# UNC-CFD/somar

Hardware: AMD Instinct MI355X
Metric: pressure-Poisson V-cycles/sec (higher is better)
Workload: dtype f64; 1 GPU; C2 single-level 512^3 Poisson, diagonal stretched metric, Neumann, LevelGSRB V-cycle 2/2/2 + BiCGStab bottom; layout = 1 box(es) 512x512x512, one per GPU; mg_depth=8, cells=134217728

## Files before the change

somar_amd/build.py:

```python
import os
import subprocess
import sys

HERE = os.path.dirname(os.path.abspath(__file__))
CSRC = os.path.join(HERE, "csrc")
OUT = os.path.join(HERE, "libsomar_amd.so")
SOURCES = ["kernels.hip", "box_bicgstab.hip", "gsrb_fused.hip", "resid_march.hip", "full19.hip", "full19_march.hip", "full19_fused.hip", "projection.hip", "line_gsrb.hip", "amr_kernels.hip", "leptic_kernels.hip", "maps.hip", "metric_refresh.hip", "box_io.hip", "tuning.cpp", "level.cpp", "solver.cpp", "solver_full.cpp", "amr.cpp", "leptic.cpp", "comm_rccl.cpp", "comm_shm.cpp", "capi.cpp"]
HEADERS = ["common.h", "devbuf.h", "tuning.h", "kernels.h", "level.h", "solver.h", "amr.h", "leptic.h", os.path.join("..", "..", "include", "somar_amd.h")]
HIPCC = os.environ.get("HIPCC", "/opt/rocm/bin/hipcc")
FLAGS = ["--offload-arch=gfx950", "-O3", "-std=c++17", "-fPIC", "-ffp-contract=off", "-fno-fast-math",
         "-Wall", "-Wno-unused-result", "-Wno-unused-value", "-I/opt/rocm/include"]


EXTRA = os.environ.get("SOMAR_EXTRA_FLAGS", "").split()


def _stale():
    if not os.path.exists(OUT):
        return True
    t = os.path.getmtime(OUT)
    return any(os.path.getmtime(os.path.join(CSRC, f)) > t for f in SOURCES + HEADERS)


def build(force=False, verbose=False):
    if not (force or _stale()):
        return OUT
    objs = []
    for f in SOURCES:
        src = os.path.join(CSRC, f)
        obj = os.path.join(CSRC, os.path.splitext(f)[0] + ".o")
        cmd = [HIPCC] + FLAGS + EXTRA + (["-x", "hip"] if f.endswith(".cpp") else []) + ["-c", src, "-o", obj]
        if verbose:
            print(" ".join(cmd))
        subprocess.check_call(cmd)
        objs.append(obj)
    cmd = [HIPCC, "--offload-arch=gfx950", "-shared", "-fPIC", "-o", OUT] + objs + ["-ldl", "-lrt"]
    if verbose:
        print(" ".join(cmd))
    subprocess.check_call(cmd)
    return OUT


if __name__ == "__main__":
    print(build(force="--force" in sys.argv, verbose=True))
```

somar_amd/csrc/gsrb_fused.hip:

```cpp
#include <type_traits>

#include "common.h"
#include "kernels.h"

namespace somar {


template <class T>
__device__ __forceinline__ T pick(const typename Vec2<T>::type& v, int s) { return s ? v.y : v.x; }

template <class T>
__device__ __forceinline__ typename Vec2<T>::type ld2(const T* __restrict__ a, long long idx, bool ok0, bool ok1,
                                                      long long safe)
{
#ifdef SOMAR_NT_LOADS
    typedef T v2d_ __attribute__((ext_vector_type(2)));
    const v2d_ w = __builtin_nontemporal_load(reinterpret_cast<const v2d_*>(a + ((ok0 || ok1) ? idx : safe)));
    const typename Vec2<T>::type v = mk2<T>(w.x, w.y);
#else
    const typename Vec2<T>::type v = *reinterpret_cast<const typename Vec2<T>::type*>(a + ((ok0 || ok1) ? idx : safe));
#endif
    return mk2<T>(ok0 ? v.x : T(0), ok1 ? v.y : T(0));
}

// ... 217 lines not shown
                        if ((p.cf & 32) && kb == p.n[2] - 1) pzh = T(P.cf_c1[2]) * own + T(P.cf_c2[2]) * zl;
                    }
                    black = gsrb_point<DIRI, INT, T>(P, xxS, yyS, zzS, p.lo[0] + li + c, gj, p.lo[2] + kb, pxl, pxh, pyl, pyh,
                                       pzl, pzh, b_gxl, b_gxh, b_gyl, b_gyh, b_gzl, pick<T>(Gzc, c), b_ji, b_rhs,
                                       Sx(sb, row, rc));
                }
                T* dst = phi_out + base + sk * kb;
                const T ox = c ? redPrev1 : black, oy = c ? black : redPrev1;
                if (out_ij[0] && out_ij[1]) *reinterpret_cast<T2*>(dst) = mk2<T>(ox, oy);
                else if (out_ij[0]) dst[0] = ox;
                else dst[1] = oy;
            }
        }

        {
            const int cb = c ^ 1;
            b_rhs = pick<T>(Rh, cb);
            b_ji = pick<T>(Ji, cb);
            b_gxl = cb ? Gx.y : Gx.x;
            b_gxh = cb ? gx_next : Gx.y;
            b_gyl = pick<T>(Gy, cb);
            b_gyh = pick<T>(Gyh, cb);
            b_gzl = pick<T>(Gzc, cb);
        }
        redPrev2 = redPrev1;
        redPrev1 = red;
        Pm = Pc;
        Pc = Pp;
        Gzc = Gzp;
    };
    const int cfirst = __builtin_amdgcn_readfirstlane((p.lo[0] + li + gj + p.lo[2] + k) & 1);
    if (cfirst) {
        for (;;) {
            if (k > kend) break;
            step(std::integral_constant<int, 1>{});
            ++k;
            if (k > kend) break;
            step(std::integral_constant<int, 0>{});
            ++k;
        }
    } else {
        for (;;) {
            if (k > kend) break;
            step(std::integral_constant<int, 0>{});
            ++k;
            if (k > kend) break;
            step(std::integral_constant<int, 1>{});
            ++k;
        }
    }
#undef Sx
}

template <int FR_J, int INMODE, bool DIRI = false, bool UNI = false, bool NARROW = false, class T = double>
__global__ __launch_bounds__(64 * FR_J) void k_gsrb_fused(const Tile* __restrict__ tiles,
                                                     const PatchDesc* __restrict__ patches,
                                                     T* __restrict__ phi_out,
                                                     const T* __restrict__ phi_in,
                                                     const T* __restrict__ rhs,
                                                     const T* __restrict__ jgx,
                                                     const T* __restrict__ jgy,
                                                     const T* __restrict__ jgz,
                                                     const T* __restrict__ jinv, StencilParams P,
                                                     const double* __restrict__ sums,
                                                     const PatchDesc* __restrict__ cpatches,
                                                     const T* __restrict__ crse, int r0, int r1, int r2, int lean_ok)
{
    __shared__ __attribute__((aligned(16))) T S[3 * FR_J * (NARROW ? 160 : 128)];
    const Tile t = tiles[blockIdx.x];
    const PatchDesc p = patches[t.patch];
    const int cls = NARROW ? t.pad_[1] : 0;
    bool lean = false;
    if (UNI && !DIRI) {
        const int wi = t.pad_[0] > 0 ? t.pad_[0] : 124;
        const int ilo = t.i0 - 1, ihi = min(t.i0 + wi, p.n[0]), jlo = t.j0 - 1, jhi = min(t.j0 + (FR_J << cls) - 4, p.n[1]);
        lean = lean_ok && p.lo[0] + ilo > P.dom_lo[0] && p.lo[0] + ihi < P.dom_hi[0] && p.lo[1] + jlo > P.dom_lo[1] &&
               p.lo[1] + jhi < P.dom_hi[1] && !((p.cf & 1) && ilo < 0) && !((p.cf & 2) && ihi >= p.n[0]) &&
               !((p.cf & 4) && jlo < 0) && !((p.cf & 8) && jhi >= p.n[1]);
    }
#define SOMAR_FUSED_BODY(INT_, CLS_)                                                                                          \
    gsrb_fused_body<FR_J, INMODE, DIRI, UNI, INT_, CLS_, T>(S, t, p, phi_out, phi_in, rhs, jgx, jgy, jgz, jinv, P, sums, cpatches, \
                                                        crse, r0, r1, r2)
    if (!NARROW || cls == 0) {
        if (lean) SOMAR_FUSED_BODY(UNI && !DIRI, 0);
        else SOMAR_FUSED_BODY(false, 0);
    } else if (cls == 1) {
        if (lean) SOMAR_FUSED_BODY(UNI && !DIRI, NARROW ? 1 : 0);
        else SOMAR_FUSED_BODY(false, NARROW ? 1 : 0);
    } else {
        SOMAR_FUSED_BODY(false, NARROW ? 4 : 0);
    }
#undef SOMAR_FUSED_BODY
}

template <class T>
static void launch_gsrb_fused_t(hipStream_t st, const Tile* tiles, int ntiles, const LevelDev& L, const MetricPtrs<T>& M,
                                T* phi_out, const T* phi_in, const T* rhs, int in_mode, const double* sums,
                                const LevelDev* C, const T* crse, const int* r)
{
    if (ntiles == 0) return;
    const PatchDesc* cpatches = C ? C->patches : nullptr;
    const int r0 = r ? r[0] : 1, r1 = r ? r[1] : 1, r2 = r ? r[2] : 1;
    SOMAR_CHECK(in_mode < 3 || ((r0 == 1 || r0 == 2) && (r1 == 1 || r1 == 2) && (r2 == 1 || r2 == 2)),
                "internal: the prolongation folded into a sweep takes multigrid ratios of 1 or 2 per direction");
    auto go = [&](auto kern, int rows) {
        hipLaunchKernelGGL(kern, dim3(ntiles), dim3(64, rows, 1), 0, st, tiles, L.patches, phi_out, phi_in, rhs, M.jg[0], M.jg[1],
                           M.jg[2], M.jinv, L.P, sums, cpatches, crse, r0, r1, r2, L.lean_tiles);
    };
#define SOMAR_FUSED_MODES(ROWS, D, U, N, M0, M1, M2, M3, M4)                    \
    switch (in_mode) {                                                          \
        case 1: go(k_gsrb_fused<ROWS, M1, D, U, N, T>, ROWS); break;            \
        case 2: go(k_gsrb_fused<ROWS, M2, D, U, N, T>, ROWS); break;            \
        case 3: go(k_gsrb_fused<ROWS, M3, D, U, N, T>, ROWS); break;            \
        case 4: go(k_gsrb_fused<ROWS, M4, D, U, N, T>, ROWS); break;            \
        default: go(k_gsrb_fused<ROWS, M0, D, U, N, T>, ROWS);                  \
    }
    const bool rows16 = L.fused_rows == 16;
    const bool narrow = L.narrow7 != 0 && rows16;
    bool diri = false;
    for (int d = 0; d < 3; ++d) diri = diri || L.P.diri[d][0] || L.P.diri[d][1];
    if (diri) {
        SOMAR_CHECK(in_mode == 0 || in_mode == 1 || in_mode == 3, "internal: mean removal on a level with Dirichlet sides");
        if (!rows16) { SOMAR_FUSED_MODES(8, true, false, false, 0, 1, 0, 3, 3) }
        else if (narrow) { SOMAR_FUSED_MODES(16, true, false, true, 0, 1, 0, 3, 3) }
        else { SOMAR_FUSED_MODES(16, true, false, false, 0, 1, 0, 3, 3) }
        return;
    }
    if (L.P.uniform && rows16) {
        if (narrow) { SOMAR_FUSED_MODES(16, false, true, true, 0, 1, 2, 3, 4) }
        else { SOMAR_FUSED_MODES(16, false, true, false, 0, 1, 2, 3, 4) }
        return;
    }
    if (!rows16) { SOMAR_FUSED_MODES(8, false, false, false, 0, 1, 2, 3, 4) }
    else if (narrow) { SOMAR_FUSED_MODES(16, false, false, true, 0, 1, 2, 3, 4) }
    else { SOMAR_FUSED_MODES(16, false, false, false, 0, 1, 2, 3, 4) }
#undef SOMAR_FUSED_MODES
}

void launch_gsrb_fused(hipStream_t st, const Tile* tiles, int ntiles, const LevelDev& L, const MetricPtrs<double>& M,
                       double* phi_out, const double* phi_in, const double* rhs, int in_mode, const double* sums,
                       const LevelDev* C, const double* crse, const int* r)
{
    launch_gsrb_fused_t<double>(st, tiles, ntiles, L, M, phi_out, phi_in, rhs, in_mode, sums, C, crse, r);
}

void launch_gsrb_fused(hipStream_t st, const Tile* tiles, int ntiles, const LevelDev& L, const MetricPtrs<float>& M,
                       float* phi_out, const float* phi_in, const float* rhs, int in_mode, const double* sums,
                       const LevelDev* C, const float* crse, const int* r)
{
    SOMAR_CHECK(fused_uniform_kernel(L) || (M.jg[0] && M.jg[1] && M.jg[2] && M.jinv),
                "internal: the fused sweep streams the metric of this depth, but its fp32 copies are missing");
    launch_gsrb_fused_t<float>(st, tiles, ntiles, L, M, phi_out, phi_in, rhs, in_mode, sums, C, crse, r);
}

bool fused_uniform_kernel(const LevelDev& L)
{
    bool diri = false;
    for (int d = 0; d < 3; ++d) diri = diri || L.P.diri[d][0] || L.P.diri[d][1];
    return L.P.uniform && L.fused_rows == 16 && !diri;
}

}
```

somar_amd/csrc/kernels.h:

```cpp
#pragma once
#include "common.h"

namespace somar {

struct LevelDev {
    const Tile* tiles = nullptr;
    int ntiles = 0;
    int tile_j = 4;
    const CopyItem* tile_items = nullptr;
    const int* tile_item_start = nullptr;
    int ghost_gy = 16;
    const PatchDesc* patches = nullptr;
    int npatches = 0;
    double* jg[3] = {nullptr, nullptr, nullptr};
    double* jinv = nullptr;
    double* lapdiag = nullptr;
    double* jgf[3][3] = {{nullptr, nullptr, nullptr}, {nullptr, nullptr, nullptr}, {nullptr, nullptr, nullptr}};
    StencilParams P;
    const double* bc_face = nullptr;
    int narrow7 = 0;
    int narrowq = 0;
    int fused_rows = 16;
    int full_rows = 8;
    int lean_tiles = 1;
    int ordered_serial = 0;
};

template <class T>
struct MetricPtrs { const T* jg[3]; const T* jinv; };
inline MetricPtrs<double> metric_ptrs(const LevelDev& L) { return MetricPtrs<double>{{L.jg[0], L.jg[1], L.jg[2]}, L.jinv}; }

struct FullFlux { const double* psi = nullptr; const double* J[3][3] = {{nullptr, nullptr, nullptr}, {nullptr, nullptr, nullptr}, {nullptr, nullptr, nullptr}}; double dxi[3] = {0, 0, 0}; };

void launch_ghost_ops(hipStream_t st, const LevelDev& L, const GhostOp* ops, int nops, double* phi, double* psi,
                      bool bc_homog = true, bool redirect = false);
void launch_ghost_ops(hipStream_t st, const LevelDev& L, const GhostOp* ops, int nops, float* phi);
void launch_ghost_program(hipStream_t st, const LevelDev& L, const GhostOp* box_ops, const int* box_first, double* phi,
                          double* psi, bool bc_homog, bool redirect, bool copy_all);
void launch_full_march(hipStream_t st, const Tile* tiles, int ntiles, const LevelDev& L, double* out, const double* phi,
                       const double* psi, const double* rhs, int mode);
void launch_gsrb_full_march(hipStream_t st, const Tile* tiles, int ntiles, const LevelDev& L, double* out,
                            const double* phi, const double* psi, const double* rhs, int color);
void launch_full_fused(hipStream_t st, const Tile* tiles, int ntiles, const LevelDev& L, double* out, const double* phi,
                       const double* psi, const double* rhs);
void launch_gsrb_full_shell(hipStream_t st, const Tile* tiles, int ntiles, const LevelDev& L, double* phi, const double* phi_in,
                            const double* psi, const double* rhs);
void launch_flux_full(hipStream_t st, const LevelDev& L, double* const out[3], const double* phi, const double* psi);
void launch_op_full(hipStream_t st, const LevelDev& L, double* out, const double* phi, const double* psi,
                    const double* rhs, int mode);
void launch_gsrb_full(hipStream_t st, const LevelDev& L, double* phi, const double* psi, const double* rhs, int color);

void launch_gsrb_ortho(hipStream_t st, const LevelDev& L, double* phi, const double* rhs, int color, int loose = 0,
                       bool pull = false);
void launch_gsrb_fused(hipStream_t st, const Tile* tiles, int ntiles, const LevelDev& L, const MetricPtrs<double>& M,
                       double* phi_out, const double* phi_in, const double* rhs, int in_mode, const double* sums,
                       const LevelDev* C, const double* crse, const int* r);
void launch_gsrb_fused(hipStream_t st, const Tile* tiles, int ntiles, const LevelDev& L, const MetricPtrs<float>& M,
                       float* phi_out, const float* phi_in, const float* rhs, int in_mode, const double* sums,
                       const LevelDev* C, const float* crse, const int* r);
bool fused_uniform_kernel(const LevelDev& L);
void launch_resid_march(hipStream_t st, const Tile* tiles, int ntiles, const LevelDev& L, double* out,
                        const double* phi, const double* rhs, int mode);
void launch_resid_restrict(hipStream_t st, const Tile* tiles, int ntiles, const LevelDev& F, const MetricPtrs<double>& M,
                           const LevelDev& C, double* crse, const double* phi, const double* rhs, const int r[3],
                           double dxProduct, double* volsum);
void launch_resid_restrict(hipStream_t st, const Tile* tiles, int ntiles, const LevelDev& F, const MetricPtrs<float>& M,
                           const LevelDev& C, float* crse, const float* phi, const float* rhs, const int r[3],
                           double dxProduct, double* volsum);
void launch_child_volume(hipStream_t st, const LevelDev& C, const LevelDev& F, double* crse, const int r[3],
                         double dxProduct);
void launch_sum_partials(hipStream_t st, const double* partials, int n, double* out);
void launch_combine_sums(hipStream_t st, double* out, const double* a, const double* b, const double* c);
void launch_line_gsrb_2d(hipStream_t st, const LevelDev& L, int maxN0, double* phi, const double* rhs, double* dmod, int color,
// ... 141 lines not shown
```

somar_amd/csrc/level.cpp:

```cpp
#include "level.h"

#include <algorithm>
#include <array>
#include <cstdlib>
#include <cstring>

namespace somar {

bool coarsenable(const std::vector<IBox>& boxes, const int* r)
{
    for (const IBox& b : boxes)
        if (!(b.coarsen(r).refine(r) == b)) return false;
    return true;
}

ExchangePlan build_exchange_plan(const IBox& domain, const bool periodic[3], const int ghost[3],
                                 const std::vector<IBox>& boxes, const std::vector<int>& owner, int myrank)
{
    ExchangePlan plan;
    std::vector<std::array<int, 3>> shifts;
    for (int a = -1; a <= 1; ++a)
        for (int b = -1; b <= 1; ++b)
            for (int cc = -1; cc <= 1; ++cc) {
                if ((a && !periodic[0]) || (b && !periodic[1]) || (cc && !periodic[2])) continue;
                shifts.push_back({a * domain.size(0), b * domain.size(1), cc * domain.size(2)});
            }
    struct Remote { int peer; CopyItem it; };
    std::vector<Remote> sends, recvs;
    for (size_t di = 0; di < boxes.size(); ++di) {
        const IBox gbox = boxes[di].grow(ghost);
        for (size_t si = 0; si < boxes.size(); ++si) {
            const bool dl = owner[di] == myrank, sl = owner[si] == myrank;
            if (!dl && !sl) continue;
            for (const auto& sh : shifts) {
                if (si == di && sh[0] == 0 && sh[1] == 0 && sh[2] == 0) continue;
                const IBox img = boxes[si].shift(sh.data());
                const IBox r = gbox & img;
                if (r.empty()) continue;
                CopyItem it;
                std::memset(&it, 0, sizeof(it));
                it.src_patch = (int)si;
                it.dst_patch = (int)di;
                for (int d = 0; d < 3; ++d) {
                    it.n[d] = r.size(d);
                    it.dst_lo[d] = r.lo[d] - boxes[di].lo[d];
                    it.src_lo[d] = r.lo[d] - sh[d] - boxes[si].lo[d];
                }
                if (dl && sl) plan.local.push_back(it);
                else if (sl) sends.push_back({owner[di], it});
                else recvs.push_back({owner[si], it});
            }
        }
    }
// ... 348 lines not shown
        if (owner[b] == myrank) plan.local.push_back(item(b));
    for (int q = 0; q < nranks; ++q) {
        if (q == myrank) continue;
        plan.peers.push_back(q);
        plan.soff.push_back(plan.send_total);
        for (size_t b = 0; b < boxes.size(); ++b)
            if (owner[b] == myrank) {
                const CopyItem it = item(b);
                plan.send_items.push_back(it);
                plan.send_itemoff.push_back(plan.send_total);
                plan.send_total += (long long)it.n[0] * it.n[1] * it.n[2];
            }
        plan.scount.push_back(plan.send_total - plan.soff.back());
        plan.roff.push_back(plan.recv_total);
        for (size_t b = 0; b < boxes.size(); ++b)
            if (owner[b] == q) {
                const CopyItem it = item(b);
                plan.recv_items.push_back(it);
                plan.recv_itemoff.push_back(plan.recv_total);
                plan.recv_total += (long long)it.n[0] * it.n[1] * it.n[2];
            }
        plan.rcount.push_back(plan.recv_total - plan.roff.back());
    }
    return plan;
}

void Copier::define_allgather(const Level& src, const Level& dst, int grow, Comm* comm)
{
    src_ = &src;
    dst_ = &dst;
    comm_ = comm;
    SOMAR_CHECK(grow >= 0 && grow <= FRAME, "allgather: ghost wider than the device frame");
    SOMAR_CHECK(dst.boxes.size() == src.boxes.size() && dst.local.size() == dst.boxes.size(),
                "allgather: the destination layout must hold every box locally");
    plan = build_allgather_plan(src.boxes, src.owner, grow, comm ? comm->rank : 0, comm ? comm->size : 1);
    std::vector<int> sp(src.boxes.size(), -1);
    for (int pi = 0; pi < (int)src.local.size(); ++pi) sp[src.local[pi]] = pi;
    for (CopyItem& it : plan.local) it.src_patch = sp[it.src_patch];
    for (CopyItem& it : plan.send_items) it.src_patch = sp[it.src_patch];
    upload_tables();
}

void Copier::run(const double* s, double* d, hipStream_t st) const
{
    const bool remote = !plan.peers.empty();
    if (remote) {
        launch_pack(st, src_->dev, d_send, d_soff, (int)plan.send_items.size(), const_cast<double*>(s), d_sbuf, true);
        comm_->neighbor_exchange(d_sbuf, d_rbuf, plan.peers, plan.soff, plan.scount, plan.roff, plan.rcount, st);
    }
    launch_copy_items2(st, src_->dev.patches, dst_->dev.patches, d_local, (int)plan.local.size(), s, d);
    if (remote) launch_pack(st, dst_->dev, d_recv, d_roff, (int)plan.recv_items.size(), d, d_rbuf, false);
}

void Level::build_march_tiles(bool narrow7)
{
    for (DevBuf<Tile>* q : {&d_ftiles, &d_ftiles_own, &d_ftiles_rem, &d_rtiles, &d_rtiles_own, &d_rtiles_rem, &d_qtiles, &d_gtiles, &d_stiles})
        q->reset();
    nftiles_own = nftiles_rem = nrtiles_own = nrtiles_rem = 0;
    narrow7_ = narrow7;
    struct ColSpec { int i0, w, cls; };
    const int fused_rows = dev.fused_rows, full_rows = dev.full_rows;
    auto march_tiles = [&](int FT_I, int region_rows, int hrows, double halo, int slots, bool classes, double min_gain = 1.0) {
        classes = classes && !tune.no_narrow_tiles;
        const bool balanced = !tune.no_balanced_tiles;
        auto columns = [&](int n0) {
            std::vector<ColSpec> eq, v;
            {
                int w = FT_I;
                if (balanced) {
                    const int ncol = (n0 + FT_I - 1) / FT_I;
                    w = (n0 + ncol - 1) / ncol;
                    w += w & 1;
                    w = std::min(w, FT_I);
                }
                for (int i0 = 0; i0 < n0; i0 += w) eq.push_back({i0, w, 0});
            }
            if (!classes || (n0 & 1)) return eq;
            int i0 = 0, rem = n0;
            double cost = 0.0;
            while (rem >= FT_I) { v.push_back({i0, FT_I, 0}); i0 += FT_I; rem -= FT_I; cost += 1.0; }
            if (rem > 76) { v.push_back({i0, rem, 0}); rem = 0; cost += 1.0; }
            if (rem > 16) { const int w = std::min(rem, 60); v.push_back({i0, w, 1}); i0 += w; rem -= w; cost += 0.5; }
            while (rem > 0) { const int w = std::min(rem, 4); v.push_back({i0, w, 4}); i0 += w; rem -= w; cost += 0.25; }
            return cost <= min_gain * (double)eq.size() ? v : eq;
        };
        auto rows_of = [&](int cls) { return (region_rows << cls) - hrows; };
        long long cols = 0;
        int maxn2 = 1;
        for (const PatchDesc& p : hpatches) {
            for (const ColSpec& c : columns(p.n[0])) cols += (p.n[1] + rows_of(c.cls) - 1) / rows_of(c.cls);
            maxn2 = std::max(maxn2, p.n[2]);
        }
        int best = 1;
        double best_eff = -1.0;
        for (int nch = 1; nch <= 64 && (nch == 1 || maxn2 / nch >= 4); ++nch) {
            const long long blocks = cols * nch;
            const long long rounds = (blocks + slots - 1) / slots;
            const double nk = (double)maxn2 / nch;
            const double eff = (double)blocks / (double)(rounds * slots) * nk / (nk + halo);
            if (eff > best_eff + 1e-9) { best_eff = eff; best = nch; }
        }
        std::vector<Tile> fnat;
        for (int pi = 0; pi < (int)hpatches.size(); ++pi) {
            const PatchDesc& p = hpatches[pi];
            int nk = (p.n[2] + best - 1) / best;
            nk += nk & 1;
            const std::vector<ColSpec> cs = columns(p.n[0]);
            auto add = [&](const ColSpec& c, int j0, int k0) {
                Tile t;
                std::memset(&t, 0, sizeof(t));
                t.patch = pi; t.i0 = c.i0; t.j0 = j0; t.k0 = k0;
                t.nk = std::min(nk, p.n[2] - k0);
                t.pad_[0] = c.w;
                t.pad_[1] = c.cls;
                fnat.push_back(t);
            };
            for (int k0 = 0; k0 < p.n[2]; k0 += nk) {
                const size_t first = fnat.size();
                for (const ColSpec& c : cs)
                    for (int j0 = 0; j0 < p.n[1]; j0 += rows_of(c.cls)) add(c, j0, k0);
                std::stable_sort(fnat.begin() + first, fnat.end(), [](const Tile& a, const Tile& b) {
                    return a.j0 != b.j0 ? a.j0 < b.j0 : a.i0 < b.i0;
                });
            }
        }
        const int NF = (int)fnat.size();
        std::vector<Tile> perm(NF);
        const int NX = 8;
        int start[NX + 1];
        start[0] = 0;
        for (int x = 0; x < NX; ++x) start[x + 1] = start[x] + (NF - x + NX - 1) / NX;
        for (int b = 0; b < NF; ++b) perm[b] = fnat[start[b % NX] + b / NX];
        return perm;
    };
    hftiles = march_tiles(124, fused_rows, 4, 3.0, 256, narrow7 && fused_rows == 16, 0.85);
    d_ftiles = DevBuf<Tile>::from(hftiles);
    nftiles = (int)hftiles.size();
    hrtiles = march_tiles(124, 16, 2, 2.0, 256, narrow7, 0.85);
    for (size_t q = 0; q < hrtiles.size(); ++q) hrtiles[q].pad_[2] = (int)q;
    d_rtiles = DevBuf<Tile>::from(hrtiles);
    nrtiles = (int)hrtiles.size();
    dev.narrow7 = 0;
    for (const Tile& t : hftiles) if (t.pad_[1]) dev.narrow7 = 1;
    hqtiles = march_tiles(124, full_rows, 2, 2.0, full_rows == 6 ? 512 : 256, full_rows == 8, 0.85);
    d_qtiles = DevBuf<Tile>::from(hqtiles);
    nqtiles = (int)hqtiles.size();
    dev.narrowq = 0;
    for (const Tile& t : hqtiles) if (t.pad_[1]) dev.narrowq = 1;
    ngtiles = nstiles = 0;
    if (want_fused19_) {
        const std::vector<Tile> g = march_tiles(124, 8, 4, 3.0, 256, false);
        d_gtiles = DevBuf<Tile>::from(g);
        ngtiles = (int)g.size();
        std::vector<Tile> sh;
        const int KC = 32;
        for (int pi = 0; pi < (int)hpatches.size(); ++pi) {
            const PatchDesc& p = hpatches[pi];
            auto add = [&](int i0, int w, int cls, int j0, int k0, int nk) {
                Tile t;
                std::memset(&t, 0, sizeof(t));
                t.patch = pi; t.i0 = i0; t.j0 = j0; t.k0 = k0; t.nk = nk;
                t.pad_[0] = w; t.pad_[1] = cls;
                sh.push_back(t);
            };
            int wcol = 124;
            {
                const int ncol = (p.n[0] + 123) / 124;
                wcol = (p.n[0] + ncol - 1) / ncol;
                wcol += wcol & 1;
                wcol = std::min(wcol, 124);
            }
            for (int k0 = 0; k0 < p.n[2]; k0 += KC) {
                const int nk = std::min(KC, p.n[2] - k0);
                for (int xi : {0, std::max(0, p.n[0] - 4)})
                    for (int j0 = 0; j0 < p.n[1]; j0 += 126) add(xi, 4, 4, j0, k0, nk);
                for (int yj : {0, std::max(0, p.n[1] - 6)})
                    for (int i0 = 0; i0 < p.n[0]; i0 += wcol) add(i0, wcol, 0, yj, k0, nk);
            }
            for (int zk : {0, std::max(0, p.n[2] - 3)})
                for (int j0 = 0; j0 < p.n[1]; j0 += 6)
                    for (int i0 = 0; i0 < p.n[0]; i0 += wcol) add(i0, wcol, 0, j0, zk, std::min(3, p.n[2] - zk));
        }
        d_stiles = DevBuf<Tile>::from(sh);
        nstiles = (int)sh.size();
    }

    if (!plan.peers.empty()) {
        std::vector<std::vector<const CopyItem*>> byDst(hpatches.size());
        for (const CopyItem& it : plan.recv_items) byDst[it.dst_patch].push_back(&it);
        auto split = [&](const std::vector<Tile>& all, int region_rows, int hrows, int halo, std::vector<Tile>& own, std::vector<Tile>& rem) {
            for (const Tile& t : all) {
                const PatchDesc& p = hpatches[t.patch];
                const int w = t.pad_[0] > 0 ? t.pad_[0] : 124;
                const int rows = (region_rows << t.pad_[1]) - hrows;
                const int lo[3] = {t.i0 - halo, t.j0 - halo, t.k0 - halo};
                const int hi[3] = {std::min(t.i0 + w, p.n[0]) - 1 + halo, std::min(t.j0 + rows, p.n[1]) - 1 + halo, t.k0 + t.nk - 1 + halo};
// ... 82 lines not shown
        for (int k0 = 0; k0 < p.n[2]; k0 += tk)
            for (int j0 = 0; j0 < p.n[1]; j0 += tj)
                for (int i0 = 0; i0 < p.n[0]; i0 += TILE_I) {
                    Tile t;
                    std::memset(&t, 0, sizeof(t));
                    t.patch = pi; t.i0 = i0; t.j0 = j0; t.k0 = k0;
                    t.nk = std::min(tk, p.n[2] - k0);
                    nat.push_back(t);
                }
    }
    const int N = (int)nat.size();
    htiles.assign(N, Tile());
    {
        const int NX = 8;
        int start[NX + 1];
        start[0] = 0;
        for (int x = 0; x < NX; ++x) start[x + 1] = start[x] + (N - x + NX - 1) / NX;
        for (int b = 0; b < N; ++b) htiles[b] = nat[start[b % NX] + b / NX];
    }

    {
        for (int pi = 0; pi < (int)hpatches.size(); ++pi) {
            const PatchDesc& p = hpatches[pi];
            for (int j0 = 0; j0 < p.n[1]; j0 += ctile_j)
                for (int i0 = 0; i0 < p.n[0]; i0 += TILE_I) {
                    Tile t;
                    std::memset(&t, 0, sizeof(t));
                    t.patch = pi; t.i0 = i0; t.j0 = j0; t.k0 = 0; t.nk = p.n[2];
                    hctiles.push_back(t);
                }
        }
        d_ctiles = DevBuf<Tile>::from(hctiles);
        nctiles = (int)hctiles.size();
    }

    int ghost[3];
    for (int d = 0; d < 3; ++d) ghost[d] = active[d] ? FRAME : 0;
    plan = build_exchange_plan(domain, periodic, ghost, boxes, owner, myrank);
    {
        std::vector<int> patch_of(boxes.size(), -1);
        for (int pi = 0; pi < (int)local.size(); ++pi) patch_of[local[pi]] = pi;
        for (CopyItem& it : plan.local) { it.src_patch = patch_of[it.src_patch]; it.dst_patch = patch_of[it.dst_patch]; }
        for (CopyItem& it : plan.send_items) it.src_patch = patch_of[it.src_patch];
        for (CopyItem& it : plan.recv_items) it.dst_patch = patch_of[it.dst_patch];
    }

    d_patches = DevBuf<PatchDesc>::from(hpatches);
    d_tiles = DevBuf<Tile>::from(htiles);
    d_local_items = DevBuf<CopyItem>::from(plan.local);
    d_send_items = DevBuf<CopyItem>::from(plan.send_items);
    d_recv_items = DevBuf<CopyItem>::from(plan.recv_items);
    d_send_off = DevBuf<long long>::from(plan.send_itemoff);
    d_recv_off = DevBuf<long long>::from(plan.recv_itemoff);
    build_march_tiles(false);
    d_sendbuf = plan.send_total ? DevBuf<double>(plan.send_total) : DevBuf<double>();
    d_recvbuf = plan.recv_total ? DevBuf<double>(plan.recv_total) : DevBuf<double>();

    dev.tiles = d_tiles;
    dev.ntiles = N;
    dev.patches = d_patches;
    dev.npatches = (int)hpatches.size();
    {
        const long long pullMax = tune.pull_max_cells;
        long long cells = 0;
        for (const IBox& b : boxes) cells += b.numPts();
        if (plan.peers.empty() && cells <= pullMax && N > 0) {
            std::vector<std::vector<int>> byDst(hpatches.size());
            for (int q = 0; q < (int)plan.local.size(); ++q) byDst[plan.local[q].dst_patch].push_back(q);
            std::vector<CopyItem> titems;
            std::vector<int> tstart(N + 1, 0);
            for (int b = 0; b < N; ++b) {
                const Tile& t = htiles[b];
                const PatchDesc& p = hpatches[t.patch];
                int lo[3] = {t.i0, t.j0, t.k0};
                int hi[3] = {std::min(t.i0 + TILE_I, p.n[0]) - 1, std::min(t.j0 + dev.tile_j, p.n[1]) - 1, t.k0 + t.nk - 1};
                for (int d = 0; d < 3; ++d)
                    if (active[d]) { lo[d] -= 1; hi[d] += 1; }
                tstart[b] = (int)titems.size();
                for (int q : byDst[t.patch]) {
                    const CopyItem& it = plan.local[q];
                    CopyItem c = it;
                    bool empty = false;
                    for (int d = 0; d < 3; ++d) {
                        const int a = std::max(lo[d], it.dst_lo[d]), e = std::min(hi[d], it.dst_lo[d] + it.n[d] - 1);
                        if (e < a) { empty = true; break; }
                        c.dst_lo[d] = a;
                        c.src_lo[d] = it.src_lo[d] + (a - it.dst_lo[d]);
                        c.n[d] = e - a + 1;
                    }
                    if (!empty) titems.push_back(c);
                }
            }
            tstart[N] = (int)titems.size();
            if (titems.empty()) titems.push_back(CopyItem());
            d_tile_items = DevBuf<CopyItem>::from(titems);
            d_tile_item_start = DevBuf<int>::from(tstart);
            dev.tile_items = d_tile_items;
            dev.tile_item_start = d_tile_item_start;
        }
    }
    {
        long long face = 0;
        for (const PatchDesc& q : hpatches) {
            const long long a = (long long)(q.n[0] + 2 * FRAME), b = (long long)(q.n[1] + 2 * FRAME), c = (long long)(q.n[2] + 2 * FRAME);
            face = std::max(face, std::max(a * b, std::max(a * c, b * c)));
        }
        dev.ghost_gy = (int)std::min<long long>(256, std::max<long long>(16, (face + 1023) / 1024));
// ... 294 lines not shown
```

somar_amd/csrc/level.h:

```cpp
#pragma once
#include <array>
#include <memory>
#include <vector>

#include "common.h"
#include "devbuf.h"
#include "kernels.h"
#include "tuning.h"

namespace somar {

struct IBox {
    int lo[3], hi[3];
    IBox() : lo{0, 0, 0}, hi{-1, -1, -1} {}
    IBox(const int* l, const int* h) { for (int d = 0; d < 3; ++d) { lo[d] = l[d]; hi[d] = h[d]; } }
    bool empty() const { return hi[0] < lo[0] || hi[1] < lo[1] || hi[2] < lo[2]; }
    int size(int d) const { return hi[d] - lo[d] + 1; }
    long long numPts() const { return empty() ? 0 : (long long)size(0) * size(1) * size(2); }
    IBox grow(const int* g) const { IBox b = *this; for (int d = 0; d < 3; ++d) { b.lo[d] -= g[d]; b.hi[d] += g[d]; } return b; }
    IBox shift(const int* s) const { IBox b = *this; for (int d = 0; d < 3; ++d) { b.lo[d] += s[d]; b.hi[d] += s[d]; } return b; }
    IBox operator&(const IBox& o) const {
        IBox b;
        for (int d = 0; d < 3; ++d) { b.lo[d] = lo[d] > o.lo[d] ? lo[d] : o.lo[d]; b.hi[d] = hi[d] < o.hi[d] ? hi[d] : o.hi[d]; }
        return b;
// ... 29 lines not shown
                                   const std::vector<long long>& soff, const std::vector<long long>& scount,
                                   const std::vector<long long>& roff, const std::vector<long long>& rcount,
                                   hipStream_t st)
    {
        (void)sendbuf; (void)recvbuf; (void)peers; (void)soff; (void)scount; (void)roff; (void)rcount; (void)st;
    }
};

struct ExchangePlan {
    std::vector<CopyItem> local;
    std::vector<int> peers;
    std::vector<CopyItem> send_items, recv_items;
    std::vector<long long> send_itemoff, recv_itemoff;
    std::vector<long long> soff, scount, roff, rcount;
    long long send_total = 0, recv_total = 0;
};

ExchangePlan build_exchange_plan(const IBox& domain, const bool periodic[3], const int ghost[3],
                                 const std::vector<IBox>& boxes, const std::vector<int>& owner, int myrank);

struct BoxIoShape {
    int ghost[3] = {0, 0, 0};
    int grow[3] = {0, 0, 0};
    int face = -1;
    int ncomp = 1;
    bool operator==(const BoxIoShape& o) const
    {
        for (int d = 0; d < 3; ++d) if (ghost[d] != o.ghost[d] || grow[d] != o.grow[d]) return false;
        return face == o.face && ncomp == o.ncomp;
    }
    static BoxIoShape cells(const int g[3], bool with_ghosts)
    {
        BoxIoShape s;
        for (int d = 0; d < 3; ++d) { s.ghost[d] = g[d]; s.grow[d] = with_ghosts ? g[d] : 0; }
        return s;
    }
    static BoxIoShape faces(int dir) { BoxIoShape s; s.face = dir; return s; }
};
void check_shape(const BoxIoShape& s);
struct BoxIoBoxes { IBox caller, region; };

class Level {
public:
    IBox domain;
    bool periodic[3] = {false, false, false};
    double dx[3] = {1, 1, 1};
    int active[3] = {1, 1, 1};
    int bc_type[3][2];
    std::vector<IBox> boxes;
    std::vector<int> owner;
    std::vector<int> local;
    std::vector<PatchDesc> hpatches;
    std::vector<Tile> htiles;
    void build_march_tiles(bool narrow7);
    bool narrow7_ = false;
    std::vector<Tile> hftiles;
    DevBuf<Tile> d_ftiles;
    int nftiles = 0;
    DevBuf<Tile> d_ftiles_own, d_ftiles_rem;
    int nftiles_own = 0, nftiles_rem = 0;
    DevBuf<Tile> d_rtiles_own, d_rtiles_rem;
    int nrtiles_own = 0, nrtiles_rem = 0;
    std::vector<Tile> hrtiles;
    DevBuf<Tile> d_rtiles;
    int nrtiles = 0;
    std::vector<Tile> hqtiles;
    DevBuf<Tile> d_qtiles;
    int nqtiles = 0;
    bool want_fused19_ = false;
    DevBuf<Tile> d_gtiles, d_stiles;
    int ngtiles = 0, nstiles = 0;
    std::vector<Tile> hctiles;
    DevBuf<Tile> d_ctiles;
    int nctiles = 0, ctile_j = 2;
    long long field_elems = 0;
    long long valid_cells_global = 0;
    ExchangePlan plan;
    Comm* comm = nullptr;
    Tuning tune;

    DevBuf<PatchDesc> d_patches;
    DevBuf<Tile> d_tiles;
    DevBuf<CopyItem> d_local_items;
    DevBuf<CopyItem> d_tile_items;
    DevBuf<int> d_tile_item_start;
    bool pull_ready() const { return bool(d_tile_item_start); }
    DevBuf<CopyItem> d_send_items, d_recv_items;
    DevBuf<long long> d_send_off, d_recv_off;
    DevBuf<double> d_sendbuf, d_recvbuf;
    DevBuf<double> jg[3], jinv, lapdiag, jgx[3][3];
    LevelDev dev;

    double alpha = 0.0, beta = 1.0;
    int mgCrseRefRatio[3] = {1, 1, 1};
    bool hasCoarser = false;
    bool zeroAvg = false;
    double dxProduct = 1.0;

    std::vector<CFCell> hcf;
    DevBuf<CFCell> d_cf;
    int ncf = 0;
    double cf_c1[3] = {0, 0, 0}, cf_c2[3] = {0, 0, 0}, cf_fac[3] = {0, 0, 0};
    std::vector<CFCell> hcfx;
    DevBuf<CFCell> d_cfx;
    int ncfx = 0;
    bool cf_fusable = true;
    std::unique_ptr<class Copier> cf_faces[3];
    void cf_homog_ext(double* phi, hipStream_t st) const
// ... 84 lines not shown
```

somar_amd/csrc/solver.cpp:

```cpp
#include "solver.h"

#include <array>
#include <chrono>
#include <cmath>
#include <cstdio>
#include <cstdlib>
#include <cstring>

namespace somar {

static const int S_MAX_COARSE = 4;
enum { SLOT_TMP = 0, SLOT_SUMS = 8, NSLOTS = 16 };

PressureSolver::PressureSolver(Comm* comm, hipStream_t shared, const Tuning& tune) : tune_(tune), comm_(comm ? comm : &self_)
{
    if (shared) { st_ = shared; own_stream_ = false; }
    else SOMAR_HIP(hipStreamCreateWithFlags(&st_, hipStreamNonBlocking));
    d_scalars = DevBuf<double>::zeros(NSLOTS);
    SOMAR_HIP(hipDeviceSynchronize());
    SOMAR_HIP(hipHostMalloc(&h_scalars, (NSLOTS + 2) * sizeof(double), hipHostMallocCoherent | hipHostMallocMapped));
    h_seq_ = reinterpret_cast<unsigned long long*>(h_scalars + NSLOTS);
    *h_seq_ = 0;
}

// ... 286 lines not shown
    xchg(L, L.dev.jinv);
}

void PressureSolver::probe_null_space(int d)
{
    Level& L = *lev[d];
    DevBuf<double> phi = L.alloc_field(), rhs0 = L.alloc_field(), res = L.alloc_field();
    launch_set(st_, phi, L.field_elems, 0.0);
    apply_op(d, rhs0, phi);
    launch_set(st_, phi, L.field_elems, 1.0);
    residual(d, res, phi, rhs0);
    launch_reduce(st_, L.dev, res, nullptr, 3, d_partials, d_scalars + SLOT_TMP);
    comm_->allreduce(d_scalars + SLOT_TMP, 1, 1, st_);
    const double maxNorm = std::fabs(fetch_scalar(SLOT_TMP));
    L.zeroAvg = maxNorm < 0.01 * (probe_eps > 0.0 ? probe_eps : prm.eps);
}

void PressureSolver::finalize()
{
    SOMAR_CHECK(!lev.empty() && !finalized, "finalize before define / twice");
    if (mp_mode_ == 1) {
        const std::string why = mixed_refusal();
        SOMAR_CHECK(why.empty(), "finalize: mixed precision (set_precision mode 1) is not available for " + why);
    }
    const bool timing = tune_.timing != 0;
    auto now = [&]() { if (timing) hipDeviceSynchronize(); return std::chrono::steady_clock::now(); };
    auto secs = [](std::chrono::steady_clock::time_point a, std::chrono::steady_clock::time_point b) {
        return std::chrono::duration<double>(b - a).count();
    };
    const auto t0 = now();
    launch_lapdiag(st_, lev[0]->dev);
    fill_metric_ghosts(*lev[0]);
    int depth = 1;
    while (build_coarser(depth)) {
        if (comm_->size > 1 && lev[depth]->valid_cells_global <= tune_.agglom_cells && !full_) {
            build_agglomerated_tail(depth);
            break;
        }
        ++depth;
    }
    const auto t1 = now();
    detect_metric_flags();
    {
        const int min_box = (int)tune_.fused19_min_box;
        fused19_.assign(lev.size(), 0);
        for (size_t d = 0; d < lev.size(); ++d) {
            Level& L = *lev[d];
            bool ok = full_ && min_box >= 0 && full_march((int)d) && tune_.full_rows == 8 && !L.boxes.empty();
            for (const IBox& b : L.boxes)
                for (int a = 0; a < 3; ++a) ok = ok && b.size(a) >= std::max(min_box, 8) && (a != 0 || b.size(a) % 2 == 0);
            fused19_[d] = ok ? 1 : 0;
            if (ok != L.want_fused19_) {
                L.want_fused19_ = ok;
                L.build_march_tiles(L.narrow7_);
            }
        }
    }
    choose_narrow_tiles();
    const auto t2 = now();
    struct Report {
        bool on; std::chrono::steady_clock::time_point t0, t1, t2; long long cells;
        ~Report() {
            if (!on) return;
            hipDeviceSynchronize();
            const auto t3 = std::chrono::steady_clock::now();
            fprintf(stderr, "[somar timing] finalize %lld cells: coarse hierarchy %.3f s, uniform detection %.3f s, fields + probes %.3f s\n",
                    cells, std::chrono::duration<double>(t1 - t0).count(), std::chrono::duration<double>(t2 - t1).count(),
                    std::chrono::duration<double>(t3 - t2).count());
        }
    } report{timing, t0, t1, t2, lev[0]->valid_cells_global};
    (void)secs;
    const int D = (int)lev.size();
    for (auto* v : {&f_res, &f_corr, &f_scratch, &f_pp}) {
        v->clear();
        v->resize(D);
    }
    if (diri_) build_face_slices();
    if (full_) {
        SOMAR_CHECK(prm.relaxMode == RELAX_LEVEL_GSRB || prm.relaxMode == RELAX_JACOBI || prm.relaxMode == RELAX_LINE_GSRB,
                    "the non-diagonal metric path offers LevelGSRB, LineGSRB and Jacobi");
        f_psi.clear();
        f_psi.resize(D);
        full_prog_.resize(D);
        for (int d = 0; d < D; ++d) {
            f_psi[d] = lev[d]->alloc_field();
            build_full_programs(d);
        }
    }
    d_diri_ops_.clear();
    d_diri_ops_.resize(D);
    n_diri_ops_.assign(D, 0);
    if (diri_)
        for (int d = 0; d < D; ++d) build_diri_ops(d);
    for (int d = 0; d < D; ++d) {
        if (d > 0) { f_res[d] = lev[d]->alloc_field(); f_corr[d] = lev[d]->alloc_field(); }
        f_scratch[d] = lev[d]->alloc_field();
        f_pp[d] = lev[d]->alloc_field();
    }
    Level& L0 = *lev[0];
    f_phi = L0.alloc_field();
    f_rhs = L0.alloc_field();
    f_uberRes = L0.alloc_field();
    f_uberCorr = L0.alloc_field();
    f_best = L0.alloc_field();
    f_W.clear();
    f_W.resize(D);
    sf_valid_.assign(D, 0);
// ... 156 lines not shown
        if (n_mm_items_) {
            d_mm_items_ = DevBuf<MinMaxItem>::from(items);
            SOMAR_HIP(hipDeviceSynchronize());
        } else d_mm_items_ = DevBuf<MinMaxItem>(1);
    }
    std::vector<double> mm(2 * (size_t)n_mm_items_ * MM_CH);
    launch_minmax_all(st_, d_mm_items_, n_mm_items_, d_mm_out_);
    if (n_mm_items_) SOMAR_HIP(hipMemcpyAsync(mm.data(), d_mm_out_, sizeof(double) * mm.size(), hipMemcpyDeviceToHost, st_));
    SOMAR_HIP(hipStreamSynchronize(st_));
    std::vector<double> h(9 * (size_t)D, -HUGE_VAL);
    for (int d = 0; d < D; ++d) {
        Level& L = *lev[d];
        const int np = L.npatches();
        double* hd = h.data() + 9 * d;
        hd[8] = (mm_first_[d] < 0 && np) ? 1.0 : 0.0;
        for (int a = 0; a < na && np && mm_first_[d] >= 0; ++a) {
            const size_t q0 = (size_t)(mm_first_[d] + a * np) * MM_CH, q1 = q0 + (size_t)np * MM_CH;
            for (size_t q = q0; q < q1; ++q) {
                if (uni_on) {
                    hd[2 * a] = std::max(hd[2 * a], mm[2 * q + 1]);
                    hd[2 * a + 1] = std::max(hd[2 * a + 1], -mm[2 * q]);
                } else {
                    if (std::isfinite(mm[2 * q])) hd[8] = std::max(hd[8], std::fabs(mm[2 * q]));
                    if (std::isfinite(mm[2 * q + 1])) hd[8] = std::max(hd[8], std::fabs(mm[2 * q + 1]));
                }
            }
        }
    }
    if (comm_->size > 1) {
        double* dh = d_mm_out_ + 2 * (size_t)std::max(n_mm_items_, 1) * MM_CH;
        SOMAR_HIP(hipMemcpyAsync(dh, h.data(), sizeof(double) * h.size(), hipMemcpyHostToDevice, st_));
        comm_->allreduce(dh, (int)h.size(), 1, st_);
        SOMAR_HIP(hipMemcpyAsync(h.data(), dh, sizeof(double) * h.size(), hipMemcpyDeviceToHost, st_));
        SOMAR_HIP(hipStreamSynchronize(st_));
    }
    for (int d = 0; d < D; ++d) {
        Level& L = *lev[d];
        if (!(L.active[0] && L.active[1] && L.active[2])) continue;
        const double* hd = h.data() + 9 * d;
        if (zero_on) { L.dev.P.zero_xy = hd[8] == 0.0 ? 1 : 0; continue; }
        bool uni = true;
        for (int a = 0; a < 4; ++a) uni = uni && std::isfinite(hd[2 * a]) && hd[2 * a] == -hd[2 * a + 1];
        if (!uni) continue;
        L.dev.P.uniform = 1;
        for (int a = 0; a < 4; ++a) L.dev.P.uc[a] = hd[2 * a];
    }
}

void PressureSolver::choose_narrow_tiles()
{
    bool rebuilt = false;
    for (auto& Lp : lev) {
        const bool want = tune_.narrow_7pt >= 0 ? tune_.narrow_7pt != 0 : Lp->dev.P.uniform != 0;
        if (want != Lp->narrow7_) { Lp->build_march_tiles(want); rebuilt = true; }
    }
    if (d_partials && !rebuilt) return;
    int maxTiles = 1;
    for (auto& L : lev) maxTiles = std::max(std::max(maxTiles, L->dev.ntiles), std::max(L->nrtiles, L->nftiles));
    SOMAR_HIP(hipStreamSynchronize(st_));
    d_partials.reset();
    d_partials = DevBuf<double>((size_t)maxTiles * 2);
}

void PressureSolver::refresh_metric()
{
    SOMAR_CHECK(finalized, "metric refresh before finalize");
    const bool timing = tune_.timing != 0;
    auto now = [&]() { if (timing) SOMAR_HIP(hipStreamSynchronize(st_)); return std::chrono::steady_clock::now(); };
    const auto t0 = now();
    const int D = (int)lev.size();
    const int nd = prm.spaceDim;
    if (d_coarsen_.empty()) {
        d_coarsen_.resize(D);
        n_coarsen_.assign(D, 0);
        gy_coarsen_.assign(D, 1);
        for (int d = 1; d < D; ++d) {
            Level& F = *lev[d - 1];
            Level& C = *lev[d];
            std::vector<CoarsenItem> items;
            long long maxGroups = 1;
            for (int pi = 0; pi < C.npatches(); ++pi) {
                auto add = [&](const double* f, double* c, int dir) {
                    items.push_back(CoarsenItem{f, c, pi, dir});
                    const int* n = C.hpatches[pi].n;
                    const long long nj = n[1] + (dir == 1), nk = n[2] + (dir == 2);
                    maxGroups = std::max(maxGroups, (nj + 3) / 4 * nk);
                };
                for (int a = 0; a < nd; ++a) add(F.dev.jg[a], C.dev.jg[a], a);
                if (full_)
                    for (int a = 0; a < nd; ++a)
                        for (int c = 0; c < nd; ++c)
                            if (c != a) add(F.dev.jgf[a][c], C.dev.jgf[a][c], a);
                add(F.dev.jinv, C.dev.jinv, -1);
            }
            n_coarsen_[d] = (int)items.size();
            gy_coarsen_[d] = (int)std::min<long long>(maxGroups, std::max<long long>(1, 8192 / std::max<int>(1, n_coarsen_[d])));
            if (!items.empty()) {
                d_coarsen_[d] = DevBuf<CoarsenItem>::from(items);
                SOMAR_HIP(hipDeviceSynchronize());
            }
        }
    }
    launch_lapdiag(st_, lev[0]->dev);
    fill_metric_ghosts(*lev[0]);
    for (int d = 1; d < D; ++d) {
        Level& F = *lev[d - 1];
        Level& C = *lev[d];
// ... 1662 lines not shown
```

Baseline: 100.2 V-cycles/s.

## Add tall class-1 tile layout for fused GSRB on non-uniform metric levels

Adds a 'tall' tiling mode for the fused GSRB sweep on levels with a non-uniform (stretched) metric. Every column becomes a class-1 tile, narrower (at most 60 wide) and twice as tall in j. The tile planner moves into a shared header and searches over extra column counts together with the k-chunk count to balance block occupancy against halo overhead. A new kernel instantiation (NARROW==2) always runs the class-1 body. The aim is better j-halo reuse and load balance on the stretched-metric case, at the cost of less i-direction coalescing per tile.

```diff
diff --git a/somar_amd/build.py b/somar_amd/build.py
--- a/somar_amd/build.py
+++ b/somar_amd/build.py
@@ -6,7 +6,7 @@
 CSRC = os.path.join(HERE, "csrc")
 OUT = os.path.join(HERE, "libsomar_amd.so")
 SOURCES = ["kernels.hip", "box_bicgstab.hip", "gsrb_fused.hip", "resid_march.hip", "full19.hip", "full19_march.hip", "full19_fused.hip", "projection.hip", "line_gsrb.hip", "amr_kernels.hip", "leptic_kernels.hip", "maps.hip", "metric_refresh.hip", "box_io.hip", "tuning.cpp", "level.cpp", "solver.cpp", "solver_full.cpp", "amr.cpp", "leptic.cpp", "comm_rccl.cpp", "comm_shm.cpp", "capi.cpp"]
-HEADERS = ["common.h", "devbuf.h", "tuning.h", "kernels.h", "level.h", "solver.h", "amr.h", "leptic.h", os.path.join("..", "..", "include", "somar_amd.h")]
+HEADERS = ["common.h", "devbuf.h", "tuning.h", "kernels.h", "level.h", "march_plan.h", "solver.h", "amr.h", "leptic.h", os.path.join("..", "..", "include", "somar_amd.h")]
 HIPCC = os.environ.get("HIPCC", "/opt/rocm/bin/hipcc")
 FLAGS = ["--offload-arch=gfx950", "-O3", "-std=c++17", "-fPIC", "-ffp-contract=off", "-fno-fast-math",
          "-Wall", "-Wno-unused-result", "-Wno-unused-value", "-I/opt/rocm/include"]
diff --git a/somar_amd/csrc/gsrb_fused.hip b/somar_amd/csrc/gsrb_fused.hip
--- a/somar_amd/csrc/gsrb_fused.hip
+++ b/somar_amd/csrc/gsrb_fused.hip
@@ -293,7 +293,7 @@
 #undef Sx
 }
 
-template <int FR_J, int INMODE, bool DIRI = false, bool UNI = false, bool NARROW = false, class T = double>
+template <int FR_J, int INMODE, bool DIRI = false, bool UNI = false, int NARROW = 0, class T = double>
 __global__ __launch_bounds__(64 * FR_J) void k_gsrb_fused(const Tile* __restrict__ tiles,
                                                      const PatchDesc* __restrict__ patches,
                                                      T* __restrict__ phi_out,
@@ -307,10 +307,10 @@
                                                      const PatchDesc* __restrict__ cpatches,
                                                      const T* __restrict__ crse, int r0, int r1, int r2, int lean_ok)
 {
-    __shared__ __attribute__((aligned(16))) T S[3 * FR_J * (NARROW ? 160 : 128)];
+    __shared__ __attribute__((aligned(16))) T S[3 * FR_J * (NARROW == 1 ? 160 : 128)];
     const Tile t = tiles[blockIdx.x];
     const PatchDesc p = patches[t.patch];
-    const int cls = NARROW ? t.pad_[1] : 0;
+    const int cls = NARROW == 1 ? t.pad_[1] : (NARROW == 2 ? 1 : 0);
     bool lean = false;
     if (UNI && !DIRI) {
         const int wi = t.pad_[0] > 0 ? t.pad_[0] : 124;
@@ -322,7 +322,9 @@
 #define SOMAR_FUSED_BODY(INT_, CLS_)                                                                                          \
     gsrb_fused_body<FR_J, INMODE, DIRI, UNI, INT_, CLS_, T>(S, t, p, phi_out, phi_in, rhs, jgx, jgy, jgz, jinv, P, sums, cpatches, \
                                                         crse, r0, r1, r2)
-    if (!NARROW || cls == 0) {
+    if constexpr (NARROW == 2) {
+        SOMAR_FUSED_BODY(false, 1);
+    } else if (!NARROW || cls == 0) {
         if (lean) SOMAR_FUSED_BODY(UNI && !DIRI, 0);
         else SOMAR_FUSED_BODY(false, 0);
     } else if (cls == 1) {
@@ -358,11 +360,14 @@
     }
     const bool rows16 = L.fused_rows == 16;
     const bool narrow = L.narrow7 != 0 && rows16;
+    const bool tall = L.tall7 != 0;
+    SOMAR_CHECK(!tall || (rows16 && !L.P.uniform), "internal: tall tiles on a level whose fused sweep has no class-1 kernel");
     bool diri = false;
     for (int d = 0; d < 3; ++d) diri = diri || L.P.diri[d][0] || L.P.diri[d][1];
     if (diri) {
         SOMAR_CHECK(in_mode == 0 || in_mode == 1 || in_mode == 3, "internal: mean removal on a level with Dirichlet sides");
         if (!rows16) { SOMAR_FUSED_MODES(8, true, false, false, 0, 1, 0, 3, 3) }
+        else if (tall) { SOMAR_FUSED_MODES(16, true, false, 2, 0, 1, 0, 3, 3) }
         else if (narrow) { SOMAR_FUSED_MODES(16, true, false, true, 0, 1, 0, 3, 3) }
         else { SOMAR_FUSED_MODES(16, true, false, false, 0, 1, 0, 3, 3) }
         return;
@@ -373,6 +378,7 @@
         return;
     }
     if (!rows16) { SOMAR_FUSED_MODES(8, false, false, false, 0, 1, 2, 3, 4) }
+    else if (tall) { SOMAR_FUSED_MODES(16, false, false, 2, 0, 1, 2, 3, 4) }
     else if (narrow) { SOMAR_FUSED_MODES(16, false, false, true, 0, 1, 2, 3, 4) }
     else { SOMAR_FUSED_MODES(16, false, false, false, 0, 1, 2, 3, 4) }
 #undef SOMAR_FUSED_MODES
diff --git a/somar_amd/csrc/kernels.h b/somar_amd/csrc/kernels.h
--- a/somar_amd/csrc/kernels.h
+++ b/somar_amd/csrc/kernels.h
@@ -19,6 +19,7 @@
     StencilParams P;
     const double* bc_face = nullptr;
     int narrow7 = 0;
+    int tall7 = 0;
     int narrowq = 0;
     int fused_rows = 16;
     int full_rows = 8;
diff --git a/somar_amd/csrc/level.cpp b/somar_amd/csrc/level.cpp
--- a/somar_amd/csrc/level.cpp
+++ b/somar_amd/csrc/level.cpp
@@ -1,4 +1,5 @@
 #include "level.h"
+#include "march_plan.h"
 
 #include <algorithm>
 #include <array>
@@ -453,60 +454,32 @@
     if (remote) launch_pack(st, dst_->dev, d_recv, d_roff, (int)plan.recv_items.size(), d, d_rbuf, false);
 }
 
-void Level::build_march_tiles(bool narrow7)
+void Level::build_march_tiles(bool narrow7, bool tall7)
 {
     for (DevBuf<Tile>* q : {&d_ftiles, &d_ftiles_own, &d_ftiles_rem, &d_rtiles, &d_rtiles_own, &d_rtiles_rem, &d_qtiles, &d_gtiles, &d_stiles})
         q->reset();
     nftiles_own = nftiles_rem = nrtiles_own = nrtiles_rem = 0;
     narrow7_ = narrow7;
-    struct ColSpec { int i0, w, cls; };
+    tall7_ = tall7;
+    using march_plan::ColSpec;
     const int fused_rows = dev.fused_rows, full_rows = dev.full_rows;
-    auto march_tiles = [&](int FT_I, int region_rows, int hrows, double halo, int slots, bool classes, double min_gain = 1.0) {
-        classes = classes && !tune.no_narrow_tiles;
-        const bool balanced = !tune.no_balanced_tiles;
-        auto columns = [&](int n0) {
-            std::vector<ColSpec> eq, v;
-            {
-                int w = FT_I;
-                if (balanced) {
-                    const int ncol = (n0 + FT_I - 1) / FT_I;
-                    w = (n0 + ncol - 1) / ncol;
-                    w += w & 1;
-                    w = std::min(w, FT_I);
-                }
-                for (int i0 = 0; i0 < n0; i0 += w) eq.push_back({i0, w, 0});
-            }
-            if (!classes || (n0 & 1)) return eq;
-            int i0 = 0, rem = n0;
-            double cost = 0.0;
-            while (rem >= FT_I) { v.push_back({i0, FT_I, 0}); i0 += FT_I; rem -= FT_I; cost += 1.0; }
-            if (rem > 76) { v.push_back({i0, rem, 0}); rem = 0; cost += 1.0; }
-            if (rem > 16) { const int w = std::min(rem, 60); v.push_back({i0, w, 1}); i0 += w; rem -= w; cost += 0.5; }
-            while (rem > 0) { const int w = std::min(rem, 4); v.push_back({i0, w, 4}); i0 += w; rem -= w; cost += 0.25; }
-            return cost <= min_gain * (double)eq.size() ? v : eq;
-        };
-        auto rows_of = [&](int cls) { return (region_rows << cls) - hrows; };
-        long long cols = 0;
-        int maxn2 = 1;
-        for (const PatchDesc& p : hpatches) {
-            for (const ColSpec& c : columns(p.n[0])) cols += (p.n[1] + rows_of(c.cls) - 1) / rows_of(c.cls);
-            maxn2 = std::max(maxn2, p.n[2]);
-        }
-        int best = 1;
-        double best_eff = -1.0;
-        for (int nch = 1; nch <= 64 && (nch == 1 || maxn2 / nch >= 4); ++nch) {
-            const long long blocks = cols * nch;
-            const long long rounds = (blocks + slots - 1) / slots;
-            const double nk = (double)maxn2 / nch;
-            const double eff = (double)blocks / (double)(rounds * slots) * nk / (nk + halo);
-            if (eff > best_eff + 1e-9) { best_eff = eff; best = nch; }
-        }
+    std::vector<march_plan::BoxSize> sizes;
+    for (const PatchDesc& p : hpatches) sizes.push_back({p.n[0], p.n[1], p.n[2]});
+    auto march_tiles = [&](int FT_I, int region_rows, int hrows, double halo, int slots, bool classes, double min_gain = 1.0,
+                           bool tall = false) {
+        march_plan::Shape shape;
+        shape.FT_I = FT_I; shape.region_rows = region_rows; shape.hrows = hrows; shape.halo = halo; shape.slots = slots;
+        shape.classes = classes && !tune.no_narrow_tiles;
+        shape.balanced = !tune.no_balanced_tiles;
+        shape.min_gain = min_gain;
+        const march_plan::Plan plan = march_plan::plan(shape, sizes, tall);
+        auto rows_of = [&](int cls) { return march_plan::rows_of(shape, cls); };
         std::vector<Tile> fnat;
         for (int pi = 0; pi < (int)hpatches.size(); ++pi) {
             const PatchDesc& p = hpatches[pi];
-            int nk = (p.n[2] + best - 1) / best;
-            nk += nk & 1;
-            const std::vector<ColSpec> cs = columns(p.n[0]);
+            const int nk = march_plan::chunk_planes(p.n[2], plan.nch);
+            const std::vector<ColSpec> cs = plan.extra >= 0 ? march_plan::tall_columns(p.n[0], plan.extra)
+                                                            : march_plan::columns(shape, p.n[0]);
             auto add = [&](const ColSpec& c, int j0, int k0) {
                 Tile t;
                 std::memset(&t, 0, sizeof(t));
@@ -534,7 +507,9 @@
         for (int b = 0; b < NF; ++b) perm[b] = fnat[start[b % NX] + b / NX];
         return perm;
     };
-    hftiles = march_tiles(124, fused_rows, 4, 3.0, 256, narrow7 && fused_rows == 16, 0.85);
+    const bool tall = tall7 && !tune.no_narrow_tiles && tune.narrow_7pt != 0 &&
+                      march_plan::tall_eligible(sizes, fused_rows, dev.P.uniform != 0);
+    hftiles = march_tiles(124, fused_rows, 4, 3.0, 256, narrow7 && fused_rows == 16, 0.85, tall);
     d_ftiles = DevBuf<Tile>::from(hftiles);
     nftiles = (int)hftiles.size();
     hrtiles = march_tiles(124, 16, 2, 2.0, 256, narrow7, 0.85);
@@ -543,6 +518,7 @@
     nrtiles = (int)hrtiles.size();
     dev.narrow7 = 0;
     for (const Tile& t : hftiles) if (t.pad_[1]) dev.narrow7 = 1;
+    dev.tall7 = tall ? 1 : 0;
     hqtiles = march_tiles(124, full_rows, 2, 2.0, full_rows == 6 ? 512 : 256, full_rows == 8, 0.85);
     d_qtiles = DevBuf<Tile>::from(hqtiles);
     nqtiles = (int)hqtiles.size();
@@ -731,7 +707,7 @@
     d_recv_items = DevBuf<CopyItem>::from(plan.recv_items);
     d_send_off = DevBuf<long long>::from(plan.send_itemoff);
     d_recv_off = DevBuf<long long>::from(plan.recv_itemoff);
-    build_march_tiles(false);
+    build_march_tiles(false, false);
     d_sendbuf = plan.send_total ? DevBuf<double>(plan.send_total) : DevBuf<double>();
     d_recvbuf = plan.recv_total ? DevBuf<double>(plan.recv_total) : DevBuf<double>();
 
diff --git a/somar_amd/csrc/level.h b/somar_amd/csrc/level.h
--- a/somar_amd/csrc/level.h
+++ b/somar_amd/csrc/level.h
@@ -105,8 +105,8 @@
     std::vector<int> local;
     std::vector<PatchDesc> hpatches;
     std::vector<Tile> htiles;
-    void build_march_tiles(bool narrow7);
-    bool narrow7_ = false;
+    void build_march_tiles(bool narrow7, bool tall7);
+    bool narrow7_ = false, tall7_ = false;
     std::vector<Tile> hftiles;
     DevBuf<Tile> d_ftiles;
     int nftiles = 0;
diff --git a/somar_amd/csrc/march_plan.h b/somar_amd/csrc/march_plan.h
--- /dev/null
+++ b/somar_amd/csrc/march_plan.h
@@ -0,0 +1,114 @@
+#pragma once
+#include <algorithm>
+#include <vector>
+
+namespace somar {
+namespace march_plan {
+
+struct ColSpec { int i0, w, cls; };
+
+struct Shape {
+    int FT_I = 124;
+    int region_rows = 16;
+    int hrows = 4;
+    double halo = 3.0;
+    int slots = 256;
+    bool classes = false;
+    bool balanced = true;
+    double min_gain = 1.0;
+};
+
+struct BoxSize { int n0, n1, n2; };
+
+inline int rows_of(const Shape& s, int cls) { return (s.region_rows << cls) - s.hrows; }
+
+inline std::vector<ColSpec> columns(const Shape& s, int n0)
+{
+    std::vector<ColSpec> eq, v;
+    {
+        int w = s.FT_I;
+        if (s.balanced) {
+            const int ncol = (n0 + s.FT_I - 1) / s.FT_I;
+            w = (n0 + ncol - 1) / ncol;
+            w += w & 1;
+            w = std::min(w, s.FT_I);
+        }
+        for (int i0 = 0; i0 < n0; i0 += w) eq.push_back({i0, w, 0});
+    }
+    if (!s.classes || (n0 & 1)) return eq;
+    int i0 = 0, rem = n0;
+    double cost = 0.0;
+    while (rem >= s.FT_I) { v.push_back({i0, s.FT_I, 0}); i0 += s.FT_I; rem -= s.FT_I; cost += 1.0; }
+    if (rem > 76) { v.push_back({i0, rem, 0}); rem = 0; cost += 1.0; }
+    if (rem > 16) { const int w = std::min(rem, 60); v.push_back({i0, w, 1}); i0 += w; rem -= w; cost += 0.5; }
+    while (rem > 0) { const int w = std::min(rem, 4); v.push_back({i0, w, 4}); i0 += w; rem -= w; cost += 0.25; }
+    return cost <= s.min_gain * (double)eq.size() ? v : eq;
+}
+
+constexpr int TALL_MAX_W = 60;
+constexpr int TALL_MIN_N0 = 128;
+
+inline bool tall_eligible(const std::vector<BoxSize>& boxes, int region_rows, bool uniform_metric)
+{
+    if (region_rows != 16 || uniform_metric || boxes.empty()) return false;
+    for (const BoxSize& b : boxes)
+        if ((b.n0 & 1) || b.n0 <= TALL_MIN_N0) return false;
+    return true;
+}
+
+inline std::vector<ColSpec> tall_columns(int n0, int extra)
+{
+    const int ncol = (n0 + TALL_MAX_W - 1) / TALL_MAX_W + extra;
+    int w = (n0 + ncol - 1) / ncol;
+    w += w & 1;
+    w = std::min(w, TALL_MAX_W);
+    std::vector<ColSpec> v;
+    for (int i0 = 0; i0 < n0; i0 += w) v.push_back({i0, w, 1});
+    return v;
+}
+
+struct Plan {
+    int nch = 1;
+    int extra = -1;
+    double eff = -1.0;
+};
+
+inline long long column_tiles(const Shape& s, const std::vector<BoxSize>& boxes, int extra)
+{
+    long long cols = 0;
+    for (const BoxSize& b : boxes)
+        for (const ColSpec& c : (extra >= 0 ? tall_columns(b.n0, extra) : columns(s, b.n0)))
+            cols += (b.n1 + rows_of(s, c.cls) - 1) / rows_of(s, c.cls);
+    return cols;
+}
+
+inline Plan plan(const Shape& s, const std::vector<BoxSize>& boxes, bool tall)
+{
+    int maxn2 = 1;
+    for (const BoxSize& b : boxes) maxn2 = std::max(maxn2, b.n2);
+    Plan best;
+    for (int extra = tall ? 0 : -1; extra <= (tall ? 2 : -1); ++extra) {
+        const long long cols = column_tiles(s, boxes, extra);
+        long long most = 0;
+        for (int nch = 1; nch <= 64 && (nch == 1 || maxn2 / nch >= 4); ++nch) {
+            const long long blocks = cols * nch;
+            const long long rounds = (blocks + s.slots - 1) / s.slots;
+            const double nk = (double)maxn2 / nch;
+            const double eff = (double)blocks / (double)(rounds * s.slots) * nk / (nk + s.halo);
+            if (eff > best.eff + 1e-9) { best.eff = eff; best.nch = nch; best.extra = extra; }
+            most = blocks;
+        }
+        if (extra == 0 && most < s.slots) break;
+    }
+    return best;
+}
+
+inline int chunk_planes(int n2, int nch)
+{
+    int nk = (n2 + nch - 1) / nch;
+    nk += nk & 1;
+    return nk;
+}
+
+}
+}
diff --git a/somar_amd/csrc/solver.cpp b/somar_amd/csrc/solver.cpp
--- a/somar_amd/csrc/solver.cpp
+++ b/somar_amd/csrc/solver.cpp
@@ -362,7 +362,7 @@
             fused19_[d] = ok ? 1 : 0;
             if (ok != L.want_fused19_) {
                 L.want_fused19_ = ok;
-                L.build_march_tiles(L.narrow7_);
+                L.build_march_tiles(L.narrow7_, L.tall7_);
             }
         }
     }
@@ -625,7 +625,8 @@
     bool rebuilt = false;
     for (auto& Lp : lev) {
         const bool want = tune_.narrow_7pt >= 0 ? tune_.narrow_7pt != 0 : Lp->dev.P.uniform != 0;
-        if (want != Lp->narrow7_) { Lp->build_march_tiles(want); rebuilt = true; }
+        const bool tall = !full_ && Lp->dev.P.uniform == 0 && Lp->active[0] && Lp->active[1] && Lp->active[2];
+        if (want != Lp->narrow7_ || tall != Lp->tall7_) { Lp->build_march_tiles(want, tall); rebuilt = true; }
     }
     if (d_partials && !rebuilt) return;
     int maxTiles = 1;
```

Result: faster. 103.6 V-cycles/s, median of 6 (+3.5%).
